# midea-ai/RDFC-GAN

Hardware: NVIDIA B200
Metric: depth maps/sec @228x304 (higher is better)
Workload: dtype bf16

## Files before the change

rdfc_gan_b200/csrc/nlspn.cu:

```cuda
#include <stdlib.h>

#include <cuda_fp16.h>

#include "common.cuh"

namespace rdfc {
namespace {

constexpr int TX = 32, TY = 8;

__device__ __forceinline__ float bilinear(const float *__restrict__ im, int H, int W, float y, float x) {
    if (!(y > -1.f && x > -1.f && y < (float)H && x < (float)W)) return 0.f;
    const float fy = floorf(y), fx = floorf(x);
    const int yl = (int)fy, xl = (int)fx;
    const float ly = y - fy, lx = x - fx, hy = 1.f - ly, hx = 1.f - lx;
    const bool y0 = yl >= 0, y1 = yl + 1 <= H - 1, x0 = xl >= 0, x1 = xl + 1 <= W - 1;
    const float *r0 = im + (long long)yl * W + xl;
    const float v1 = (y0 && x0) ? __ldg(r0) : 0.f;
    const float v2 = (y0 && x1) ? __ldg(r0 + 1) : 0.f;
    const float v3 = (y1 && x0) ? __ldg(r0 + W) : 0.f;
    const float v4 = (y1 && x1) ? __ldg(r0 + W + 1) : 0.f;
    return hy * hx * v1 + hy * lx * v2 + ly * hx * v3 + ly * lx * v4;
}

template <bool kPacked>
__global__ void __launch_bounds__(TX *TY) nlspn_affinity_kernel(const float *__restrict__ guidance,
                                                                const float *__restrict__ confidence,
                                                                const float *__restrict__ conv_w,
                                                                const float *__restrict__ conv_b,
                                                                const float *__restrict__ aff_scale, int affinity,
                                                                int conf_prop, float *__restrict__ offset,
                                                                float *__restrict__ aff, uint4 *__restrict__ packed, int H, int W) {
    __shared__ __align__(16) float s_w[72 * 24];
    __shared__ float s_b[24];
    __shared__ float s_g[8][TY + 2][TX + 2];
    const int tid = threadIdx.y * TX + threadIdx.x;
    const int b = blockIdx.z, x0 = blockIdx.x * TX, y0 = blockIdx.y * TY;
    const long long P = (long long)H * W;
    for (int e = tid; e < 24 * 72; e += TX * TY) s_w[(e % 72) * 24 + e / 72] = conv_w[e];
    if (tid < 24) s_b[tid] = conv_b[tid];
    for (int e = tid; e < 8 * (TY + 2) * (TX + 2); e += TX * TY) {
        const int c = e / ((TY + 2) * (TX + 2)), r = e % ((TY + 2) * (TX + 2));
        const int yy = y0 + r / (TX + 2) - 1, xx = x0 + r % (TX + 2) - 1;
        s_g[c][r / (TX + 2)][r % (TX + 2)] =
            (yy >= 0 && yy < H && xx >= 0 && xx < W) ? __ldg(guidance + ((long long)b * 8 + c) * P + (long long)yy * W + xx) : 0.f;
    }
    __syncthreads();
    const int x = x0 + threadIdx.x, y = y0 + threadIdx.y;
    if (x >= W || y >= H) return;

    float o[24];
#pragma unroll
    for (int c = 0; c < 24; ++c) o[c] = s_b[c];
#pragma unroll
    for (int ci = 0; ci < 8; ++ci)
#pragma unroll
        for (int t = 0; t < 9; ++t) {
            const float g = s_g[ci][threadIdx.y + t / 3][threadIdx.x + t % 3];
            const float4 *w4 = reinterpret_cast<const float4 *>(s_w + (ci * 9 + t) * 24);
#pragma unroll
            for (int c4 = 0; c4 < 6; ++c4) {
                const float4 w = w4[c4];
                o[4 * c4 + 0] = fmaf(w.x, g, o[4 * c4 + 0]);
                o[4 * c4 + 1] = fmaf(w.y, g, o[4 * c4 + 1]);
                o[4 * c4 + 2] = fmaf(w.z, g, o[4 * c4 + 2]);
                o[4 * c4 + 3] = fmaf(w.w, g, o[4 * c4 + 3]);
            }
        }

    const float scale = __ldg(aff_scale);
    float a[8];
    float abs_sum = 0.f;
    const float *conf = confidence + (long long)b * P;
#pragma unroll
    for (int j = 0; j < 8; ++j) {
        float v = o[16 + j];
        if (affinity == RDFC_AFF_TC) v = tanhf(v) / scale;
        else if (affinity == RDFC_AFF_TGASS) v = tanhf(v) / (scale + 1e-8f);
        if (conf_prop) v *= bilinear(conf, H, W, (float)y + o[2 * j], (float)x + o[2 * j + 1]);
        a[j] = v;
        abs_sum += fabsf(v);
    }
    abs_sum += 1e-4f;
    if (affinity == RDFC_AFF_ASS || affinity == RDFC_AFF_TGASS) abs_sum = abs_sum < 1.f ? 1.f : abs_sum;
    float sum = 0.f;
#pragma unroll
    for (int j = 0; j < 8; ++j) {
        if (affinity != RDFC_AFF_TC) a[j] = a[j] / abs_sum;
        sum += a[j];
    }
    const long long pix = (long long)y * W + x;
    if (kPacked) {
        const long long g = (long long)b * P + pix;
        uint4 *p = packed + (g >> 5) * 96 + (g & 31);
        auto h2 = [](float a_, float b_) { const __half2 h = __floats2half2_rn(a_, b_); return *reinterpret_cast<const uint32_t *>(&h); };
        p[0] = make_uint4(h2(o[0], o[1]), h2(o[2], o[3]), h2(o[4], o[5]), h2(o[6], o[7]));
        p[32] = make_uint4(h2(o[8], o[9]), h2(o[10], o[11]), h2(o[12], o[13]), h2(o[14], o[15]));
        p[64] = make_uint4(h2(a[0], a[1]), h2(a[2], a[3]), h2(a[4], a[5]), h2(a[6], a[7]));
        return;
    }
    float *offp = offset + (long long)b * 18 * P + pix;
    float *affp = aff + (long long)b * 9 * P + pix;
#pragma unroll
    for (int j = 0; j < 8; ++j) {
        const int k = j < 4 ? j : j + 1;
        offp[(long long)(2 * k) * P] = o[2 * j];
        offp[(long long)(2 * k + 1) * P] = o[2 * j + 1];
        affp[(long long)k * P] = a[j];
    }
    offp[8 * P] = 0.f;
    offp[9 * P] = 0.f;
    affp[4 * P] = 1.f - sum;
}

struct FuseOut { const float *d1, *c1, *c2; float *pred; };

__device__ __forceinline__ float feat_at(const float *__restrict__ im, const float *__restrict__ fix, long long i) {
    float v = __ldg(im + i);
    if (fix) {
        const float f = __ldg(fix + i);
        v = f > 0.f ? f : v;
    }
    return v;
}

__device__ __forceinline__ float bilinear_fix(const float *__restrict__ im, const float *__restrict__ fix, int H, int W, float y, float x) {
    if (!(y > -1.f && x > -1.f && y < (float)H && x < (float)W)) return 0.f;
    const float fy = floorf(y), fx = floorf(x);
    const int yl = (int)fy, xl = (int)fx;
    const float ly = y - fy, lx = x - fx, hy = 1.f - ly, hx = 1.f - lx;
    const bool y0 = yl >= 0, y1 = yl + 1 <= H - 1, x0 = xl >= 0, x1 = xl + 1 <= W - 1;
    const long long i = (long long)yl * W + xl;
    const float v1 = (y0 && x0) ? feat_at(im, fix, i) : 0.f;
    const float v2 = (y0 && x1) ? feat_at(im, fix, i + 1) : 0.f;
    const float v3 = (y1 && x0) ? feat_at(im, fix, i + W) : 0.f;
    const float v4 = (y1 && x1) ? feat_at(im, fix, i + W + 1) : 0.f;
    return hy * hx * v1 + hy * lx * v2 + ly * hx * v3 + ly * lx * v4;
}

struct BandView {
    const float *tile;
    const float *im, *fix;
    int pitch, ty0, nrows, H, W;
    float Hf, Wf;
};

template <typename FDy, typename FDx, typename FA>
__device__ __forceinline__ float gather9(const BandView &v, FDy dyf, FDx dxf, FA af, int y, int x) {
    float ymin = 1e30f, ymax = -1e30f;
#pragma unroll
    for (int k = 0; k < 9; ++k) {
        const float cy = fminf(fmaxf((float)(y - 1 + k / 3) + dyf(k), -1.f), v.Hf);
        ymin = fminf(ymin, cy);
        ymax = fmaxf(ymax, cy);
    }
    const bool esc = ((int)floorf(ymin) < v.ty0) | ((int)floorf(ymax) + 1 >= v.ty0 + v.nrows);
    float acc = 0.f;
    if (!esc) {
#pragma unroll
        for (int k = 0; k < 9; ++k) {
            const float cy = fminf(fmaxf((float)(y - 1 + k / 3) + dyf(k), -1.f), v.Hf);
            const float cx = fminf(fmaxf((float)(x - 1 + k % 3) + dxf(k), -1.f), v.Wf);
            const float fy = floorf(cy), fx = floorf(cx);
            const float ly = cy - fy, lx = cx - fx, hy = 1.f - ly, hx = 1.f - lx;
            const float *q = v.tile + (int)fmaf(fy - (float)v.ty0, (float)v.pitch, fx + 1.f);
            acc = fmaf(af(k), hy * hx * q[0] + hy * lx * q[1] + ly * hx * q[v.pitch] + ly * lx * q[v.pitch + 1], acc);
        }
    } else {
#pragma unroll
        for (int k = 0; k < 9; ++k)
            acc = fmaf(af(k), bilinear_fix(v.im, v.fix, v.H, v.W, (float)(y - 1 + k / 3) + dyf(k), (float)(x - 1 + k % 3) + dxf(k)), acc);
    }
    return acc;
}

constexpr int BAND_THREADS = 256;

__device__ __forceinline__ void stage_band(float *tile, const float *__restrict__ im, const float *__restrict__ fix, int ty0, int nrows,
                                           int pitch, int H, int W) {
    const int warp = threadIdx.x >> 5, lane = threadIdx.x & 31;
    for (int tr = warp; tr < nrows; tr += BAND_THREADS / 32) {
        const int iy = ty0 + tr;
        const bool yok = iy >= 0 && iy < H;
        const long long base = (long long)iy * W - 1;
        float *dst = tile + tr * pitch;
        for (int tc = lane; tc < pitch; tc += 32) dst[tc] = (yok && tc >= 1 && tc <= W) ? feat_at(im, fix, base + tc) : 0.f;
    }
}

template <bool kFinal>
__device__ __forceinline__ float finish(float acc, int clamp, const FuseOut &fz, long long o) {
    if (kFinal) {
        if (clamp) acc = fminf(fmaxf(acc, -1.f), 1.f);
        if (fz.pred) {
            const float a = __ldg(fz.c1 + o), b = __ldg(fz.c2 + o), m = fmaxf(a, b);
            const float e1 = expf(a - m), e2 = expf(b - m), inv = 1.f / (e1 + e2);
            fz.pred[o] = __ldg(fz.d1 + o) * (e1 * inv) + acc * (e2 * inv);
        }
    }
    return acc;
}

__device__ __forceinline__ float ld_stream(const float *p) {
    float v;
    asm volatile("ld.global.nc.L1::no_allocate.f32 %0, [%1];" : "=f"(v) : "l"(p));
    return v;
}
__device__ __forceinline__ float2 ld_stream2(const float *p) {
    float2 v;
    asm volatile("ld.global.nc.L1::no_allocate.v2.f32 {%0, %1}, [%2];" : "=f"(v.x), "=f"(v.y) : "l"(p));
    return v;
}
__device__ __forceinline__ uint4 ld_stream4(const uint4 *p) {
    uint4 v;
    asm volatile("ld.global.nc.L1::no_allocate.v4.u32 {%0, %1, %2, %3}, [%4];" : "=r"(v.x), "=r"(v.y), "=r"(v.z), "=r"(v.w) : "l"(p));
    return v;
}

template <bool kFinal, int kPix, int kMinBlocks>
__global__ void __launch_bounds__(BAND_THREADS, kMinBlocks)
nlspn_prop_band_kernel(const float *__restrict__ in, const float *__restrict__ offset, const float *__restrict__ aff,
                       const float *__restrict__ fixp, float *__restrict__ out, float *__restrict__ inter, FuseOut fz, int clamp,
                       int B, int H, int W, int rows_per_cta, int sub_rows, int halo, int pitch) {
    extern __shared__ float band_tile[];
    const long long total = (long long)B * H, P = (long long)H * W;
    long long row = (long long)blockIdx.x * rows_per_cta;
    const long long row_end = row + rows_per_cta < total ? row + rows_per_cta : total;
    const int Wp = W / kPix;
    const float Hf = (float)H, Wf = (float)W;
    asm volatile("griddepcontrol.launch_dependents;" ::: "memory");
    asm volatile("griddepcontrol.wait;" ::: "memory");
    while (row < row_end) {
        const int b = (int)(row / H), y_lo = (int)(row - (long long)b * H);
        long long nrl = row_end - row;
        if (nrl > H - y_lo) nrl = H - y_lo;
        if (nrl > sub_rows) nrl = sub_rows;
        const int nr = (int)nrl;
        const int ty0 = y_lo - halo - 1;
        const int nrows = nr + 2 * halo + 3;
        const float *im = in + (long long)b * P;
        const float *fix = fixp ? fixp + (long long)b * P : nullptr;
        __syncthreads();
        stage_band(band_tile, im, fix, ty0, nrows, pitch, H, W);
        __syncthreads();
        const BandView bv{band_tile, im, fix, pitch, ty0, nrows, H, W, Hf, Wf};
        const int nitems = nr * Wp;
        for (int idx = threadIdx.x; idx < nitems; idx += BAND_THREADS) {
            const int ry = idx / Wp, x = kPix * (idx - ry * Wp), y = y_lo + ry;
            const long long pix = (long long)y * W + x;
            const float *offp = offset + (long long)b * 18 * P + pix;
            const float *affp = aff + (long long)b * 9 * P + pix;
            const long long o = (long long)b * P + pix;
            if (kPix == 2) {
                float2 a[9], dy[9], dx[9];
#pragma unroll
                for (int k = 0; k < 9; ++k) {
                    a[k] = ld_stream2(affp + (long long)k * P);
                    if (k == 4) {
                        dy[k] = dx[k] = make_float2(0.f, 0.f);
                    } else {
                        dy[k] = ld_stream2(offp + (long long)(2 * k) * P);
                        dx[k] = ld_stream2(offp + (long long)(2 * k + 1) * P);
                    }
                }
                float acc0 = gather9(bv, [&](int k) { return dy[k].x; }, [&](int k) { return dx[k].x; }, [&](int k) { return a[k].x; }, y, x);
                float acc1 = gather9(bv, [&](int k) { return dy[k].y; }, [&](int k) { return dx[k].y; }, [&](int k) { return a[k].y; }, y, x + 1);
                acc0 = finish<kFinal>(acc0, clamp, fz, o);
                acc1 = finish<kFinal>(acc1, clamp, fz, o + 1);
                *reinterpret_cast<float2 *>(out + o) = make_float2(acc0, acc1);
                if (inter) *reinterpret_cast<float2 *>(inter + o) = make_float2(acc0, acc1);
            } else {
                float a[9], dy[9], dx[9];
#pragma unroll
                for (int k = 0; k < 9; ++k) {
                    a[k] = ld_stream(affp + (long long)k * P);
                    if (k == 4) {
                        dy[k] = dx[k] = 0.f;
                    } else {
                        dy[k] = ld_stream(offp + (long long)(2 * k) * P);
                        dx[k] = ld_stream(offp + (long long)(2 * k + 1) * P);
                    }
                }
                float acc = gather9(bv, [&](int k) { return dy[k]; }, [&](int k) { return dx[k]; }, [&](int k) { return a[k]; }, y, x);
                acc = finish<kFinal>(acc, clamp, fz, o);
                out[o] = acc;
                if (inter) inter[o] = acc;
            }
        }
        row += nr;
    }
}

__device__ __forceinline__ float2 h2f(uint32_t u) {
    const __half2 h = *reinterpret_cast<const __half2 *>(&u);
    return __half22float2(h);
}

template <bool kFinal>
__global__ void __launch_bounds__(BAND_THREADS, 4)
nlspn_prop_packed_kernel(const float *__restrict__ in, const uint4 *__restrict__ pk, const float *__restrict__ fixp,
                         float *__restrict__ out, FuseOut fz, int clamp, int B, int H, int W, int rows_per_cta, int sub_rows, int halo, int pitch) {
    extern __shared__ float band_tile[];
    const long long total = (long long)B * H, P = (long long)H * W;
    long long row = (long long)blockIdx.x * rows_per_cta;
    const long long row_end = row + rows_per_cta < total ? row + rows_per_cta : total;
    const float Hf = (float)H, Wf = (float)W;
    asm volatile("griddepcontrol.launch_dependents;" ::: "memory");
    asm volatile("griddepcontrol.wait;" ::: "memory");
    while (row < row_end) {
        const int b = (int)(row / H), y_lo = (int)(row - (long long)b * H);
        long long nrl = row_end - row;
        if (nrl > H - y_lo) nrl = H - y_lo;
        if (nrl > sub_rows) nrl = sub_rows;
        const int nr = (int)nrl;
        const int ty0 = y_lo - halo - 1;
        const int nrows = nr + 2 * halo + 3;
        const float *im = in + (long long)b * P;
        const float *fix = fixp ? fixp + (long long)b * P : nullptr;
        __syncthreads();
        stage_band(band_tile, im, fix, ty0, nrows, pitch, H, W);
        __syncthreads();
        const BandView bv{band_tile, im, fix, pitch, ty0, nrows, H, W, Hf, Wf};
        const long long g0 = (long long)b * P + (long long)y_lo * W, g1 = g0 + (long long)nr * W;
        long long g = (g0 & ~31ll) + threadIdx.x;
        uint4 n0 = make_uint4(0, 0, 0, 0), n1 = n0, n2 = n0;
        if (g < g1) { const uint4 *p = pk + (g >> 5) * 96 + (g & 31); n0 = ld_stream4(p); n1 = ld_stream4(p + 32); n2 = ld_stream4(p + 64); }
        for (; g < g1; g += BAND_THREADS) {
            const uint4 c0 = n0, c1 = n1, c2 = n2;
            if (g + BAND_THREADS < g1) {
                const uint4 *p = pk + ((g + BAND_THREADS) >> 5) * 96 + ((g + BAND_THREADS) & 31);
                n0 = ld_stream4(p); n1 = ld_stream4(p + 32); n2 = ld_stream4(p + 64);
            }
            if (g < g0) continue;
            const int pix = (int)(g - (long long)b * P), y = pix / W, x = pix - y * W;
            float dy[9], dx[9], a[9];
            {
                float2 t;
                t = h2f(c0.x); dy[0] = t.x; dx[0] = t.y;
                t = h2f(c0.y); dy[1] = t.x; dx[1] = t.y;
                t = h2f(c0.z); dy[2] = t.x; dx[2] = t.y;
                t = h2f(c0.w); dy[3] = t.x; dx[3] = t.y;
                dy[4] = dx[4] = 0.f;
                t = h2f(c1.x); dy[5] = t.x; dx[5] = t.y;
                t = h2f(c1.y); dy[6] = t.x; dx[6] = t.y;
                t = h2f(c1.z); dy[7] = t.x; dx[7] = t.y;
                t = h2f(c1.w); dy[8] = t.x; dx[8] = t.y;
                t = h2f(c2.x); a[0] = t.x; a[1] = t.y;
                t = h2f(c2.y); a[2] = t.x; a[3] = t.y;
                t = h2f(c2.z); a[5] = t.x; a[6] = t.y;
                t = h2f(c2.w); a[7] = t.x; a[8] = t.y;
                a[4] = 1.f - (((a[0] + a[1]) + (a[2] + a[3])) + ((a[5] + a[6]) + (a[7] + a[8])));
            }
            float acc = gather9(bv, [&](int k) { return dy[k]; }, [&](int k) { return dx[k]; }, [&](int k) { return a[k]; }, y, x);
            acc = finish<kFinal>(acc, clamp, fz, g);
            out[g] = acc;
        }
        row += nr;
    }
}

template <bool kFinal>
__global__ void __launch_bounds__(TX *TY) nlspn_prop_kernel(const float *__restrict__ in, const float *__restrict__ offset,
                                                            const float *__restrict__ aff, const float *__restrict__ fixp,
                                                            float *__restrict__ out, float *__restrict__ inter, FuseOut fz, int clamp,
                                                            int H, int W) {
    const int x = blockIdx.x * TX + threadIdx.x, y = blockIdx.y * TY + threadIdx.y, b = blockIdx.z;
    if (x >= W || y >= H) return;
    const long long P = (long long)H * W, pix = (long long)y * W + x;
    const float *offp = offset + (long long)b * 18 * P + pix;
    const float *affp = aff + (long long)b * 9 * P + pix;
    const float *im = in + (long long)b * P;
    const float *fix = fixp ? fixp + (long long)b * P : nullptr;
    float dy[9], dx[9], a[9];
#pragma unroll
    for (int k = 0; k < 9; ++k) {
        a[k] = ld_stream(affp + (long long)k * P);
        dy[k] = k == 4 ? 0.f : ld_stream(offp + (long long)(2 * k) * P);
        dx[k] = k == 4 ? 0.f : ld_stream(offp + (long long)(2 * k + 1) * P);
    }
    float acc = 0.f;
#pragma unroll
    for (int k = 0; k < 9; ++k)
        acc = fmaf(a[k], bilinear_fix(im, fix, H, W, (float)(y - 1 + k / 3) + dy[k], (float)(x - 1 + k % 3) + dx[k]), acc);
    acc = finish<kFinal>(acc, clamp, fz, (long long)b * P + pix);
    out[(long long)b * P + pix] = acc;
    if (inter) inter[(long long)b * P + pix] = acc;
}

__global__ void fuse_depth_kernel(const float *__restrict__ d1, const float *__restrict__ c1,
                                  const float *__restrict__ d2, const float *__restrict__ c2,
                                  float *__restrict__ d2c, float *__restrict__ pred, size_t n) {
    for (size_t i = (size_t)blockIdx.x * blockDim.x + threadIdx.x; i < n; i += (size_t)gridDim.x * blockDim.x) {
        const float v2 = fminf(fmaxf(d2[i], -1.f), 1.f);
        const float a = c1[i], b = c2[i], m = fmaxf(a, b);
        const float e1 = expf(a - m), e2 = expf(b - m), inv = 1.f / (e1 + e2);
        if (d2c) d2c[i] = v2;
        pred[i] = d1[i] * (e1 * inv) + v2 * (e2 * inv);
    }
}

static int band_pitch(int W) { return knob("RDFC_NLSPN_PITCH32", 1) != 0 ? (W + 4 + 31) / 32 * 32 : W + 4; }

struct BandGeom { int per_sm, rows_per_cta, sub_rows, nctas; size_t smem; bool ok; };
static BandGeom band_geom(int B, int H, int W, int halo, int per_sm_max) {
    BandGeom g{};
    const long long total = (long long)B * H;
    const size_t row_bytes = (size_t)band_pitch(W) * sizeof(float);
    for (int per_sm = per_sm_max; per_sm >= 1; --per_sm) {
        const size_t cap = (size_t)(220 * 1024) / per_sm - 1024;
        int fit = (int)(cap / row_bytes) - 2 * halo - 3;
        if (const long long sub = knob("RDFC_NLSPN_SUB", 0); sub > 0 && fit > sub && per_sm == per_sm_max) fit = (int)sub;
        if (fit < (per_sm > 1 && knob("RDFC_NLSPN_SUB", 0) <= 0 ? 12 : 1)) continue;
        long long ctas = (long long)sm_count() * per_sm;
        if (ctas > total) ctas = total;
        g.per_sm = per_sm;
        g.rows_per_cta = (int)((total + ctas - 1) / ctas);
        g.sub_rows = fit < g.rows_per_cta ? fit : g.rows_per_cta;
        if (g.sub_rows > H) g.sub_rows = H;
        g.nctas = (int)((total + g.rows_per_cta - 1) / g.rows_per_cta);
        g.smem = (size_t)(g.sub_rows + 2 * halo + 3) * row_bytes;
        g.ok = true;
        return g;
    }
    return g;
}

template <typename Kern, typename... Args>
static cudaError_t launch_pdl(Kern kern, int grid, int block, size_t smem, cudaStream_t st, int pdl, Args... args) {
    cudaLaunchConfig_t cfg = {};
    cfg.gridDim = dim3(grid); cfg.blockDim = dim3(block); cfg.dynamicSmemBytes = smem; cfg.stream = st;
    cudaLaunchAttribute attr[1];
    attr[0].id = cudaLaunchAttributeProgrammaticStreamSerialization;
    attr[0].val.programmaticStreamSerializationAllowed = pdl;
    cfg.attrs = attr; cfg.numAttrs = 1;
    return cudaLaunchKernelEx(&cfg, kern, args...);
}

static size_t packed_bytes(int B, int H, int W) { return (size_t)(((long long)B * H * W + 31) / 32) * 1536; }

}
}

using namespace rdfc;

static int affinity_check(const void *guidance, const void *confidence, const void *conv_w, const void *conv_b, const void *aff_scale,
                          int affinity, int conf_prop, int B, int H, int W) {
    RDFC_REQUIRE(guidance && conv_w && conv_b && aff_scale, "NULL pointer argument");
    RDFC_REQUIRE(!conf_prop || confidence, "conf_prop requires a confidence map (nlspn_model.py:150-151)");
    RDFC_REQUIRE(B > 0 && H > 0 && W > 0 && B <= 65535, "bad shape (%d,%d,%d)", B, H, W);
    RDFC_REQUIRE(affinity >= RDFC_AFF_AS && affinity <= RDFC_AFF_TGASS, "unknown affinity mode %d", affinity);
    return 0;
}

extern "C" int rdfc_nlspn_affinity_forward(const float *guidance, const float *confidence, const float *conv_w,
                                           const float *conv_b, const float *aff_scale, int affinity, int conf_prop,
                                           float *offset, float *aff, int B, int H, int W, void *stream) {
    if (int rc = affinity_check(guidance, confidence, conv_w, conv_b, aff_scale, affinity, conf_prop, B, H, W)) return rc;
    RDFC_REQUIRE(offset && aff, "NULL output pointer");
    dim3 grid(cdiv(W, TX), cdiv(H, TY), B), block(TX, TY);
    nlspn_affinity_kernel<false><<<grid, block, 0, (cudaStream_t)stream>>>(guidance, confidence, conv_w, conv_b, aff_scale,
                                                                            affinity, conf_prop, offset, aff, nullptr, H, W);
    RDFC_CHECK_LAUNCH("nlspn_affinity_kernel");
    return 0;
}

extern "C" size_t rdfc_nlspn_packed_bytes(int B, int H, int W) { return (B > 0 && H > 0 && W > 0) ? packed_bytes(B, H, W) : 0; }

extern "C" int rdfc_nlspn_affinity_forward_packed(const float *guidance, const float *confidence, const float *conv_w,
                                                  const float *conv_b, const float *aff_scale, int affinity, int conf_prop,
                                                  void *packed, int B, int H, int W, void *stream) {
    if (int rc = affinity_check(guidance, confidence, conv_w, conv_b, aff_scale, affinity, conf_prop, B, H, W)) return rc;
    RDFC_REQUIRE(packed && ((uintptr_t)packed % 16) == 0, "packed stream must be a 16-byte aligned buffer of rdfc_nlspn_packed_bytes()");
    dim3 grid(cdiv(W, TX), cdiv(H, TY), B), block(TX, TY);
    nlspn_affinity_kernel<true><<<grid, block, 0, (cudaStream_t)stream>>>(guidance, confidence, conv_w, conv_b, aff_scale,
                                                                           affinity, conf_prop, nullptr, nullptr, (uint4 *)packed, H, W);
    RDFC_CHECK_LAUNCH("nlspn_affinity_kernel");
    return 0;
}

static int propagate(const float *feat_init, const float *offset, const float *aff, const void *packed, const float *feat_fix,
                     int preserve_input, float *out, float *scratch, float *inter, int B, int H, int W, int prop_time, int clamp_out,
                     const rdfc_fuse_out *fuse, cudaStream_t st) {
    RDFC_REQUIRE(feat_init && out && scratch, "NULL pointer argument");
    RDFC_REQUIRE(!preserve_input || feat_fix, "preserve_input requires feat_fix (nlspn_model.py:157-158)");
    RDFC_REQUIRE(B > 0 && H > 0 && W > 0 && prop_time >= 0, "bad shape (%d,%d,%d) x %d", B, H, W, prop_time);
    RDFC_REQUIRE(!fuse || (fuse->d1 && fuse->c1 && fuse->c2 && fuse->pred), "fuse: NULL pointer");
    const long long P = (long long)H * W;
    const FuseOut fz = fuse ? FuseOut{fuse->d1, fuse->c1, fuse->c2, fuse->pred} : FuseOut{nullptr, nullptr, nullptr, nullptr};
    const int clamp = (clamp_out || fuse) ? 1 : 0;
    if (prop_time == 0) {
        if (fuse) {
            const int nblk = (int)min((long long)cdiv(B * P, 256), (long long)sm_count() * 8);
            fuse_depth_kernel<<<nblk, 256, 0, st>>>(fuse->d1, fuse->c1, feat_init, fuse->c2, out, fuse->pred, (size_t)(B * P));
            RDFC_CHECK_LAUNCH("fuse_depth_kernel");
        } else {
            RDFC_CUDA(cudaMemcpyAsync(out, feat_init, sizeof(float) * B * P, cudaMemcpyDeviceToDevice, st));
        }
        return 0;
    }
    const float *fix = preserve_input ? feat_fix : nullptr;
    const int halo = (int)knob("RDFC_NLSPN_HALO", 6);
    const int pdl = knob("RDFC_NLSPN_PDL", 1) != 0;
    const bool simple = knob("RDFC_NLSPN_SIMPLE", 0) != 0;
    const int pix = (!packed && W % 2 == 0 && P % 2 == 0 && ((uintptr_t)offset % 8) == 0 && ((uintptr_t)aff % 8) == 0 &&
                     ((uintptr_t)out % 8) == 0 && ((uintptr_t)scratch % 8) == 0 && (!inter || ((uintptr_t)inter % 8) == 0)) ? 2 : 1;
    const int per_sm_max = (int)knob("RDFC_NLSPN_PER_SM", packed ? 4 : (pix == 2 ? 3 : 5));
    const BandGeom g = band_geom(B, H, W, halo, per_sm_max);
    const bool band = g.ok && !simple;
    RDFC_REQUIRE(band || !packed, "packed NLSPN stream: image too wide for the band kernel (W = %d)", W);
    if (band) {
        if (packed) {
            RDFC_CUDA(cudaFuncSetAttribute(nlspn_prop_packed_kernel<false>, cudaFuncAttributeMaxDynamicSharedMemorySize, 220 * 1024));
            RDFC_CUDA(cudaFuncSetAttribute(nlspn_prop_packed_kernel<true>, cudaFuncAttributeMaxDynamicSharedMemorySize, 220 * 1024));
        } else if (pix == 2) {
            RDFC_CUDA(cudaFuncSetAttribute(nlspn_prop_band_kernel<false, 2, 3>, cudaFuncAttributeMaxDynamicSharedMemorySize, 220 * 1024));
            RDFC_CUDA(cudaFuncSetAttribute(nlspn_prop_band_kernel<true, 2, 3>, cudaFuncAttributeMaxDynamicSharedMemorySize, 220 * 1024));
        } else {
            RDFC_CUDA(cudaFuncSetAttribute(nlspn_prop_band_kernel<false, 1, 5>, cudaFuncAttributeMaxDynamicSharedMemorySize, 220 * 1024));
            RDFC_CUDA(cudaFuncSetAttribute(nlspn_prop_band_kernel<true, 1, 5>, cudaFuncAttributeMaxDynamicSharedMemorySize, 220 * 1024));
        }
    }
    float *bufs[2] = {scratch, out};
    const float *cur = feat_init;
    for (int t = 0; t < prop_time; ++t) {
        float *dst = bufs[(prop_time - 1 - t) % 2 == 0 ? 1 : 0];
        float *it = inter ? inter + (long long)t * B * P : nullptr;
        const bool last = t == prop_time - 1;
        const FuseOut none{nullptr, nullptr, nullptr, nullptr};
        if (band && packed) {
            if (last) RDFC_CUDA(launch_pdl(nlspn_prop_packed_kernel<true>, g.nctas, BAND_THREADS, g.smem, st, pdl, cur, (const uint4 *)packed, fix, dst, fz, clamp, B, H, W, g.rows_per_cta, g.sub_rows, halo, band_pitch(W)));
            else RDFC_CUDA(launch_pdl(nlspn_prop_packed_kernel<false>, g.nctas, BAND_THREADS, g.smem, st, pdl, cur, (const uint4 *)packed, fix, dst, none, 0, B, H, W, g.rows_per_cta, g.sub_rows, halo, band_pitch(W)));
            RDFC_CHECK_LAUNCH("nlspn_prop_packed_kernel");
        } else if (band) {
#define RDFC_BAND(FIN, PX, MB, FZ, CL)                                                                                            \
    RDFC_CUDA(launch_pdl(nlspn_prop_band_kernel<FIN, PX, MB>, g.nctas, BAND_THREADS, g.smem, st, pdl, cur, offset, aff, fix, dst, it, \
                         FZ, CL, B, H, W, g.rows_per_cta, g.sub_rows, halo, band_pitch(W)))
            if (pix == 2) { if (last) RDFC_BAND(true, 2, 3, fz, clamp); else RDFC_BAND(false, 2, 3, none, 0); }
            else { if (last) RDFC_BAND(true, 1, 5, fz, clamp); else RDFC_BAND(false, 1, 5, none, 0); }
#undef RDFC_BAND
            RDFC_CHECK_LAUNCH("nlspn_prop_band_kernel");
        } else {
            RDFC_REQUIRE(B <= 65535, "batch too large for the fallback kernel");
            dim3 grid(cdiv(W, TX), cdiv(H, TY), B), block(TX, TY);
            if (last) nlspn_prop_kernel<true><<<grid, block, 0, st>>>(cur, offset, aff, fix, dst, it, fz, clamp, H, W);
            else nlspn_prop_kernel<false><<<grid, block, 0, st>>>(cur, offset, aff, fix, dst, it, none, 0, H, W);
            RDFC_CHECK_LAUNCH("nlspn_prop_kernel");
        }
        cur = dst;
    }
    return 0;
}

extern "C" int rdfc_nlspn_propagate_forward(const float *feat_init, const float *offset, const float *aff,
                                            const float *feat_fix, int preserve_input, float *out, float *scratch,
                                            float *inter, int B, int H, int W, int prop_time, int clamp_out,
                                            const rdfc_fuse_out *fuse, void *stream) {
    RDFC_REQUIRE(offset && aff, "NULL pointer argument");
    return propagate(feat_init, offset, aff, nullptr, feat_fix, preserve_input, out, scratch, inter, B, H, W, prop_time, clamp_out,
                     fuse, (cudaStream_t)stream);
}

extern "C" int rdfc_nlspn_propagate_forward_packed(const float *feat_init, const void *packed, const float *feat_fix,
                                                   int preserve_input, float *out, float *scratch, int B, int H, int W,
                                                   int prop_time, int clamp_out, const rdfc_fuse_out *fuse, void *stream) {
    RDFC_REQUIRE(packed && ((uintptr_t)packed % 16) == 0, "packed stream must be 16-byte aligned");
    return propagate(feat_init, nullptr, nullptr, packed, feat_fix, preserve_input, out, scratch, nullptr, B, H, W, prop_time,
                     clamp_out, fuse, (cudaStream_t)stream);
}

__global__ void __launch_bounds__(TX *TY) nlspn_affinity_bwd_kernel(const float *__restrict__ guidance, const float *__restrict__ confidence,
                                                                    const float *__restrict__ conv_w, const float *__restrict__ conv_b,
                                                                    const float *__restrict__ aff_scale, int affinity, int conf_prop,
                                                                    const float *__restrict__ offset, const float *__restrict__ g_offset,
                                                                    const float *__restrict__ g_aff, float *__restrict__ g_conv,
                                                                    float *__restrict__ g_conf, float *__restrict__ g_scale, int H, int W) {
    __shared__ __align__(16) float s_w[72 * 8];
    __shared__ float s_b[8];
    __shared__ float s_g[8][TY + 2][TX + 2];
    __shared__ float s_red[TX * TY / 32];
    const int tid = threadIdx.y * TX + threadIdx.x;
    const int b = blockIdx.z, x0 = blockIdx.x * TX, y0 = blockIdx.y * TY;
    const long long P = (long long)H * W;
    for (int e = tid; e < 8 * 72; e += TX * TY) s_w[(e % 72) * 8 + e / 72] = conv_w[16 * 72 + e];
    if (tid < 8) s_b[tid] = conv_b[16 + tid];
    for (int e = tid; e < 8 * (TY + 2) * (TX + 2); e += TX * TY) {
        const int c = e / ((TY + 2) * (TX + 2)), r = e % ((TY + 2) * (TX + 2));
        const int yy = y0 + r / (TX + 2) - 1, xx = x0 + r % (TX + 2) - 1;
        s_g[c][r / (TX + 2)][r % (TX + 2)] =
            (yy >= 0 && yy < H && xx >= 0 && xx < W) ? __ldg(guidance + ((long long)b * 8 + c) * P + (long long)yy * W + xx) : 0.f;
    }
    __syncthreads();
    const int x = x0 + threadIdx.x, y = y0 + threadIdx.y;
    const bool live = x < W && y < H;
    float gs = 0.f;
    if (live) {
        float r[8];
#pragma unroll
        for (int j = 0; j < 8; ++j) r[j] = s_b[j];
#pragma unroll
        for (int ci = 0; ci < 8; ++ci)
#pragma unroll
            for (int t = 0; t < 9; ++t) {
                const float g = s_g[ci][threadIdx.y + t / 3][threadIdx.x + t % 3];
                const float4 *w4 = reinterpret_cast<const float4 *>(s_w + (ci * 9 + t) * 8);
                const float4 w0 = w4[0], w1 = w4[1];
                r[0] = fmaf(w0.x, g, r[0]); r[1] = fmaf(w0.y, g, r[1]); r[2] = fmaf(w0.z, g, r[2]); r[3] = fmaf(w0.w, g, r[3]);
                r[4] = fmaf(w1.x, g, r[4]); r[5] = fmaf(w1.y, g, r[5]); r[6] = fmaf(w1.z, g, r[6]); r[7] = fmaf(w1.w, g, r[7]);
            }
        const long long pix = (long long)y * W + x;
        const float *offp = offset + (long long)b * 18 * P + pix;
        const float *gop = g_offset + (long long)b * 18 * P + pix;
        const float *gap = g_aff + (long long)b * 9 * P + pix;
        float *gc = g_conv + (long long)b * 24 * P + pix;
        const float scale = __ldg(aff_scale);
        const float den = affinity == RDFC_AFF_TGASS ? scale + 1e-8f : scale;
        const float *conf = conf_prop ? confidence + (long long)b * P : nullptr;
        float t[8], v[8], c[8], u[8], dy[8], dx[8];
        float abs_sum = 0.f;
#pragma unroll
        for (int j = 0; j < 8; ++j) {
            const int k = j < 4 ? j : j + 1;
            dy[j] = __ldg(offp + (long long)(2 * k) * P);
            dx[j] = __ldg(offp + (long long)(2 * k + 1) * P);
            t[j] = (affinity == RDFC_AFF_TC || affinity == RDFC_AFF_TGASS) ? tanhf(r[j]) : r[j];
            v[j] = (affinity == RDFC_AFF_TC || affinity == RDFC_AFF_TGASS) ? t[j] / den : r[j];
            c[j] = conf_prop ? bilinear(conf, H, W, (float)y + dy[j], (float)x + dx[j]) : 1.f;
            u[j] = v[j] * c[j];
            abs_sum += fabsf(u[j]);
        }
        abs_sum += 1e-4f;
        bool clamped = false;
        if ((affinity == RDFC_AFF_ASS || affinity == RDFC_AFF_TGASS) && abs_sum < 1.f) { abs_sum = 1.f; clamped = true; }
        const float g_ref = __ldg(gap + 4 * P);
        float ga[8], dot = 0.f;
#pragma unroll
        for (int j = 0; j < 8; ++j) {
            const int k = j < 4 ? j : j + 1;
            ga[j] = __ldg(gap + (long long)k * P) - g_ref;
            dot += ga[j] * u[j];
        }
#pragma unroll
        for (int j = 0; j < 8; ++j) {
            float gu = ga[j];
            if (affinity != RDFC_AFF_TC) {
                const float sgn = u[j] > 0.f ? 1.f : (u[j] < 0.f ? -1.f : 0.f);
                gu = ga[j] / abs_sum - (clamped ? 0.f : dot / (abs_sum * abs_sum) * sgn);
            }
            const float gv = gu * c[j];
            if (conf_prop) {
                const float gcj = gu * v[j], sy = (float)y + dy[j], sx = (float)x + dx[j];
                if (gcj != 0.f && sy > -1.f && sx > -1.f && sy < (float)H && sx < (float)W) {
                    const float fy = floorf(sy), fx = floorf(sx);
                    const int yl = (int)fy, xl = (int)fx;
                    const float ly = sy - fy, lx = sx - fx;
                    float *gim = g_conf + (long long)b * P;
#pragma unroll
                    for (int aa = 0; aa < 2; ++aa)
#pragma unroll
                        for (int cc = 0; cc < 2; ++cc) {
                            const int yy = yl + aa, xx = xl + cc;
                            if (yy >= 0 && yy <= H - 1 && xx >= 0 && xx <= W - 1)
                                atomicAdd(gim + (long long)yy * W + xx, (aa ? ly : 1.f - ly) * (cc ? lx : 1.f - lx) * gcj);
                        }
                }
            }
            float gr = gv;
            if (affinity == RDFC_AFF_TC || affinity == RDFC_AFF_TGASS) {
                gr = gv * (1.f - t[j] * t[j]) / den;
                gs -= gv * t[j] / (den * den);
            }
            gc[(long long)(16 + j) * P] = gr;
            const int k = j < 4 ? j : j + 1;
            gc[(long long)(2 * j) * P] = __ldg(gop + (long long)(2 * k) * P);
            gc[(long long)(2 * j + 1) * P] = __ldg(gop + (long long)(2 * k + 1) * P);
        }
    }
    if (g_scale) {
        for (int o = 16; o > 0; o >>= 1) gs += __shfl_down_sync(0xffffffffu, gs, o);
        if ((tid & 31) == 0) s_red[tid >> 5] = gs;
        __syncthreads();
        if (tid == 0) {
            float tot = 0.f;
            for (int w = 0; w < TX * TY / 32; ++w) tot += s_red[w];
            if (tot != 0.f) atomicAdd(g_scale, tot);
        }
    }
}

struct BwdPos { int yl, xl; float ly, lx; bool valid; };
__device__ __forceinline__ BwdPos bwd_pos(float y, float x, int H, int W) {
    BwdPos q;
    q.valid = y > -1.f && x > -1.f && y < (float)H && x < (float)W;
    const float yf = floorf(y), xf = floorf(x);
    q.yl = (int)yf; q.xl = (int)xf; q.ly = y - yf; q.lx = x - xf;
    return q;
}

__global__ void __launch_bounds__(256) nlspn_bwd_scatter_kernel(float *__restrict__ g, const float *__restrict__ ginter,
                                                                const float *__restrict__ fix, const float *__restrict__ offset,
                                                                const float *__restrict__ aff, float *__restrict__ gprev,
                                                                int finalize, int H, int W) {
    const long long P = (long long)H * W;
    const int b = blockIdx.y;
    const long long pix = (long long)blockIdx.x * 256 + threadIdx.x;
    if (pix >= P) return;
    const long long o = (long long)b * P + pix;
    float gv = g[o];
    if (finalize) {
        if (fix && __ldg(fix + o) > 0.f) gv = 0.f;
        if (ginter) gv += __ldg(ginter + o);
        g[o] = gv;
    }
    if (gv == 0.f) return;
    const int y = (int)(pix / W), x = (int)(pix - (long long)y * W);
    const float *offp = offset + (long long)b * 18 * P + pix;
    const float *affp = aff + (long long)b * 9 * P + pix;
    float *gim = gprev + (long long)b * P;
#pragma unroll
    for (int k = 0; k < 9; ++k) {
        const float sy = (float)(y - 1 + k / 3) + __ldg(offp + (long long)(2 * k) * P);
        const float sx = (float)(x - 1 + k % 3) + __ldg(offp + (long long)(2 * k + 1) * P);
        const BwdPos q = bwd_pos(sy, sx, H, W);
        if (!q.valid) continue;
        const float top = gv * __ldg(affp + (long long)k * P);
#pragma unroll
        for (int a = 0; a < 2; ++a)
#pragma unroll
            for (int c = 0; c < 2; ++c) {
                const int yy = q.yl + a, xx = q.xl + c;
                if (yy >= 0 && yy <= H - 1 && xx >= 0 && xx <= W - 1)
                    atomicAdd(gim + (long long)yy * W + xx, (a ? q.ly : 1.f - q.ly) * (c ? q.lx : 1.f - q.lx) * top);
            }
    }
}

template <bool kPreserve>
__global__ void __launch_bounds__(256) nlspn_bwd_coord_kernel(const float *__restrict__ feat_init, const float *__restrict__ inter,
                                                              const float *__restrict__ fix, const float *__restrict__ G,
                                                              const float *__restrict__ offset, const float *__restrict__ aff,
                                                              float *__restrict__ goff, float *__restrict__ gaff,
                                                              int B, int H, int W, int T) {
    const long long P = (long long)H * W, BP = (long long)B * P;
    const int b = blockIdx.y;
    const long long pix = (long long)blockIdx.x * 256 + threadIdx.x;
    if (pix >= P) return;
    const long long o = (long long)b * P + pix;
    const int y = (int)(pix / W), x = (int)(pix - (long long)y * W);
    const float *offp = offset + (long long)b * 18 * P + pix;
    const float *affp = aff + (long long)b * 9 * P + pix;
    const float *fx = kPreserve ? fix + (long long)b * P : nullptr;
#pragma unroll 1
    for (int k = 0; k < 9; ++k) {
        const float sy = (float)(y - 1 + k / 3) + __ldg(offp + (long long)(2 * k) * P);
        const float sx = (float)(x - 1 + k % 3) + __ldg(offp + (long long)(2 * k + 1) * P);
        const float m = __ldg(affp + (long long)k * P);
        float a_m = 0.f, a_y = 0.f, a_x = 0.f;
        if (!(sy <= -1.f || sy >= (float)H || sx <= -1.f || sx >= (float)W)) {
            const BwdPos q = bwd_pos(sy, sx, H, W);
            const int yh = q.yl + 1, xh = q.xl + 1;
            const bool ok1 = q.yl >= 0 && q.xl >= 0, ok2 = q.yl >= 0 && xh <= W - 1, ok3 = yh <= H - 1 && q.xl >= 0,
                       ok4 = yh <= H - 1 && xh <= W - 1;
            const long long i1 = (long long)q.yl * W + q.xl, i2 = i1 + 1, i3 = i1 + W, i4 = i3 + 1;
            const float hy = 1.f - q.ly, hx = 1.f - q.lx;
            for (int t = 1; t <= T; ++t) {
                const float gv = __ldg(G + (long long)t * BP + o);
                if (gv == 0.f) continue;
                const float *im = (t == 1 ? feat_init : inter + (long long)(t - 2) * BP) + (long long)b * P;
                float v1 = ok1 ? __ldg(im + i1) : 0.f, v2 = ok2 ? __ldg(im + i2) : 0.f, v3 = ok3 ? __ldg(im + i3) : 0.f,
                      v4 = ok4 ? __ldg(im + i4) : 0.f;
                if (kPreserve) {
                    const float f1 = ok1 ? __ldg(fx + i1) : 0.f, f2 = ok2 ? __ldg(fx + i2) : 0.f, f3 = ok3 ? __ldg(fx + i3) : 0.f,
                                f4 = ok4 ? __ldg(fx + i4) : 0.f;
                    v1 = f1 > 0.f ? f1 : v1; v2 = f2 > 0.f ? f2 : v2; v3 = f3 > 0.f ? f3 : v3; v4 = f4 > 0.f ? f4 : v4;
                }
                const float val = hy * hx * v1 + hy * q.lx * v2 + q.ly * hx * v3 + q.ly * q.lx * v4;
                a_m += gv * val;
// ... 82 lines not shown
```

Before: 2957.

## Use packed FP32x2 math in NLSPN affinity conv and deformable gather paths

The affinity kernel now computes two pixels per thread with paired FFMA2 instructions, and it prefetches weights and guidance into registers before writing them to shared memory. The propagation gather adds a fast path for when all vertical offsets fall within the halo, which skips the band-escape min/max check. That path samples two taps at once using packed float2 add/multiply and a magic-number floor. Band staging is batched so several loads are in flight per lane. These changes cut instruction count and load latency, in exchange for more register pressure and integer-bit tricks in floor/address computation that could be fragile at edge values.

```diff
diff --git a/rdfc_gan_b200/csrc/nlspn.cu b/rdfc_gan_b200/csrc/nlspn.cu
--- a/rdfc_gan_b200/csrc/nlspn.cu
+++ b/rdfc_gan_b200/csrc/nlspn.cu
@@ -23,6 +23,60 @@
     return hy * hx * v1 + hy * lx * v2 + ly * hx * v3 + ly * lx * v4;
 }
 
+constexpr int AX = 2 * TX;
+
+template <bool kPacked>
+__device__ __forceinline__ void affinity_epilogue(const float2 (&o2)[12], const float *__restrict__ conf, float scale, int affinity,
+                                                  int conf_prop, float *__restrict__ offset, float *__restrict__ aff,
+                                                  uint4 *__restrict__ packed, int b, int H, int W, int y, int x, bool store) {
+    const long long P = (long long)H * W;
+    float o[24];
+#pragma unroll
+    for (int c = 0; c < 12; ++c) { o[2 * c] = o2[c].x; o[2 * c + 1] = o2[c].y; }
+    float a[8];
+    float abs_sum = 0.f;
+#pragma unroll
+    for (int j = 0; j < 8; ++j) {
+        float v = o[16 + j];
+        if (affinity == RDFC_AFF_TC) v = tanhf(v) / scale;
+        else if (affinity == RDFC_AFF_TGASS) v = tanhf(v) / (scale + 1e-8f);
+        if (conf_prop) v *= bilinear(conf, H, W, (float)y + o[2 * j], (float)x + o[2 * j + 1]);
+        a[j] = v;
+        abs_sum += fabsf(v);
+    }
+    abs_sum += 1e-4f;
+    if (affinity == RDFC_AFF_ASS || affinity == RDFC_AFF_TGASS) abs_sum = abs_sum < 1.f ? 1.f : abs_sum;
+    float sum = 0.f;
+#pragma unroll
+    for (int j = 0; j < 8; ++j) {
+        if (affinity != RDFC_AFF_TC) a[j] = a[j] / abs_sum;
+        sum += a[j];
+    }
+    if (!store) return;
+    const long long pix = (long long)y * W + x;
+    if (kPacked) {
+        const long long g = (long long)b * P + pix;
+        uint4 *p = packed + (g >> 5) * 96 + (g & 31);
+        auto h2 = [](float a_, float b_) { const __half2 h = __floats2half2_rn(a_, b_); return *reinterpret_cast<const uint32_t *>(&h); };
+        p[0] = make_uint4(h2(o[0], o[1]), h2(o[2], o[3]), h2(o[4], o[5]), h2(o[6], o[7]));
+        p[32] = make_uint4(h2(o[8], o[9]), h2(o[10], o[11]), h2(o[12], o[13]), h2(o[14], o[15]));
+        p[64] = make_uint4(h2(a[0], a[1]), h2(a[2], a[3]), h2(a[4], a[5]), h2(a[6], a[7]));
+        return;
+    }
+    float *offp = offset + (long long)b * 18 * P + pix;
+    float *affp = aff + (long long)b * 9 * P + pix;
+#pragma unroll
+    for (int j = 0; j < 8; ++j) {
+        const int k = j < 4 ? j : j + 1;
+        offp[(long long)(2 * k) * P] = o[2 * j];
+        offp[(long long)(2 * k + 1) * P] = o[2 * j + 1];
+        affp[(long long)k * P] = a[j];
+    }
+    offp[8 * P] = 0.f;
+    offp[9 * P] = 0.f;
+    affp[4 * P] = 1.f - sum;
+}
+
 template <bool kPacked>
 __global__ void __launch_bounds__(TX *TY) nlspn_affinity_kernel(const float *__restrict__ guidance,
                                                                 const float *__restrict__ confidence,
@@ -33,84 +87,65 @@
                                                                 float *__restrict__ aff, uint4 *__restrict__ packed, int H, int W) {
     __shared__ __align__(16) float s_w[72 * 24];
     __shared__ float s_b[24];
-    __shared__ float s_g[8][TY + 2][TX + 2];
+    __shared__ __align__(8) float s_g[8][TY + 2][AX + 2];
     const int tid = threadIdx.y * TX + threadIdx.x;
-    const int b = blockIdx.z, x0 = blockIdx.x * TX, y0 = blockIdx.y * TY;
+    const int b = blockIdx.z, x0 = blockIdx.x * AX, y0 = blockIdx.y * TY;
     const long long P = (long long)H * W;
-    for (int e = tid; e < 24 * 72; e += TX * TY) s_w[(e % 72) * 24 + e / 72] = conv_w[e];
+    constexpr int NW = 24 * 72, NG = 8 * (TY + 2) * (AX + 2), NT = TX * TY;
+    float wv[(NW + NT - 1) / NT], gv[(NG + NT - 1) / NT];
+#pragma unroll
+    for (int i = 0; i < (NW + NT - 1) / NT; ++i) wv[i] = tid + i * NT < NW ? __ldg(conv_w + tid + i * NT) : 0.f;
+#pragma unroll
+    for (int i = 0; i < (NG + NT - 1) / NT; ++i) {
+        const int e = tid + i * NT, c = e / ((TY + 2) * (AX + 2)), r = e % ((TY + 2) * (AX + 2));
+        const int yy = y0 + r / (AX + 2) - 1, xx = x0 + r % (AX + 2) - 1;
+        gv[i] = (e < NG && yy >= 0 && yy < H && xx >= 0 && xx < W) ? __ldg(guidance + ((long long)b * 8 + c) * P + (long long)yy * W + xx) : 0.f;
+    }
     if (tid < 24) s_b[tid] = conv_b[tid];
-    for (int e = tid; e < 8 * (TY + 2) * (TX + 2); e += TX * TY) {
-        const int c = e / ((TY + 2) * (TX + 2)), r = e % ((TY + 2) * (TX + 2));
-        const int yy = y0 + r / (TX + 2) - 1, xx = x0 + r % (TX + 2) - 1;
-        s_g[c][r / (TX + 2)][r % (TX + 2)] =
-            (yy >= 0 && yy < H && xx >= 0 && xx < W) ? __ldg(guidance + ((long long)b * 8 + c) * P + (long long)yy * W + xx) : 0.f;
+#pragma unroll
+    for (int i = 0; i < (NW + NT - 1) / NT; ++i) {
+        const int e = tid + i * NT;
+        if (e < NW) s_w[(e % 72) * 24 + e / 72] = wv[i];
+    }
+#pragma unroll
+    for (int i = 0; i < (NG + NT - 1) / NT; ++i) {
+        const int e = tid + i * NT;
+        if (e < NG) (&s_g[0][0][0])[e] = gv[i];
     }
     __syncthreads();
-    const int x = x0 + threadIdx.x, y = y0 + threadIdx.y;
+    const int x = x0 + 2 * threadIdx.x, y = y0 + threadIdx.y;
     if (x >= W || y >= H) return;
 
-    float o[24];
-#pragma unroll
-    for (int c = 0; c < 24; ++c) o[c] = s_b[c];
+    float2 o0[12], o1[12];
+#pragma unroll
+    for (int c = 0; c < 12; ++c) o0[c] = o1[c] = make_float2(s_b[2 * c], s_b[2 * c + 1]);
 #pragma unroll
     for (int ci = 0; ci < 8; ++ci)
 #pragma unroll
-        for (int t = 0; t < 9; ++t) {
-            const float g = s_g[ci][threadIdx.y + t / 3][threadIdx.x + t % 3];
-            const float4 *w4 = reinterpret_cast<const float4 *>(s_w + (ci * 9 + t) * 24);
-#pragma unroll
-            for (int c4 = 0; c4 < 6; ++c4) {
-                const float4 w = w4[c4];
-                o[4 * c4 + 0] = fmaf(w.x, g, o[4 * c4 + 0]);
-                o[4 * c4 + 1] = fmaf(w.y, g, o[4 * c4 + 1]);
-                o[4 * c4 + 2] = fmaf(w.z, g, o[4 * c4 + 2]);
-                o[4 * c4 + 3] = fmaf(w.w, g, o[4 * c4 + 3]);
+        for (int ky = 0; ky < 3; ++ky) {
+            const float2 *row = reinterpret_cast<const float2 *>(&s_g[ci][threadIdx.y + ky][2 * threadIdx.x]);
+            const float2 ga = row[0], gb = row[1];
+            const float g[4] = {ga.x, ga.y, gb.x, gb.y};
+#pragma unroll
+            for (int kx = 0; kx < 3; ++kx) {
+                const float4 *w4 = reinterpret_cast<const float4 *>(s_w + (ci * 9 + ky * 3 + kx) * 24);
+                const float2 g0 = make_float2(g[kx], g[kx]), g1 = make_float2(g[kx + 1], g[kx + 1]);
+#pragma unroll
+                for (int c4 = 0; c4 < 6; ++c4) {
+                    const float4 w = w4[c4];
+                    const float2 wl = make_float2(w.x, w.y), wh = make_float2(w.z, w.w);
+                    o0[2 * c4] = __ffma2_rn(wl, g0, o0[2 * c4]);
+                    o0[2 * c4 + 1] = __ffma2_rn(wh, g0, o0[2 * c4 + 1]);
+                    o1[2 * c4] = __ffma2_rn(wl, g1, o1[2 * c4]);
+                    o1[2 * c4 + 1] = __ffma2_rn(wh, g1, o1[2 * c4 + 1]);
+                }
             }
         }
 
     const float scale = __ldg(aff_scale);
-    float a[8];
-    float abs_sum = 0.f;
     const float *conf = confidence + (long long)b * P;
-#pragma unroll
-    for (int j = 0; j < 8; ++j) {
-        float v = o[16 + j];
-        if (affinity == RDFC_AFF_TC) v = tanhf(v) / scale;
-        else if (affinity == RDFC_AFF_TGASS) v = tanhf(v) / (scale + 1e-8f);
-        if (conf_prop) v *= bilinear(conf, H, W, (float)y + o[2 * j], (float)x + o[2 * j + 1]);
-        a[j] = v;
-        abs_sum += fabsf(v);
-    }
-    abs_sum += 1e-4f;
-    if (affinity == RDFC_AFF_ASS || affinity == RDFC_AFF_TGASS) abs_sum = abs_sum < 1.f ? 1.f : abs_sum;
-    float sum = 0.f;
-#pragma unroll
-    for (int j = 0; j < 8; ++j) {
-        if (affinity != RDFC_AFF_TC) a[j] = a[j] / abs_sum;
-        sum += a[j];
-    }
-    const long long pix = (long long)y * W + x;
-    if (kPacked) {
-        const long long g = (long long)b * P + pix;
-        uint4 *p = packed + (g >> 5) * 96 + (g & 31);
-        auto h2 = [](float a_, float b_) { const __half2 h = __floats2half2_rn(a_, b_); return *reinterpret_cast<const uint32_t *>(&h); };
-        p[0] = make_uint4(h2(o[0], o[1]), h2(o[2], o[3]), h2(o[4], o[5]), h2(o[6], o[7]));
-        p[32] = make_uint4(h2(o[8], o[9]), h2(o[10], o[11]), h2(o[12], o[13]), h2(o[14], o[15]));
-        p[64] = make_uint4(h2(a[0], a[1]), h2(a[2], a[3]), h2(a[4], a[5]), h2(a[6], a[7]));
-        return;
-    }
-    float *offp = offset + (long long)b * 18 * P + pix;
-    float *affp = aff + (long long)b * 9 * P + pix;
-#pragma unroll
-    for (int j = 0; j < 8; ++j) {
-        const int k = j < 4 ? j : j + 1;
-        offp[(long long)(2 * k) * P] = o[2 * j];
-        offp[(long long)(2 * k + 1) * P] = o[2 * j + 1];
-        affp[(long long)k * P] = a[j];
-    }
-    offp[8 * P] = 0.f;
-    offp[9 * P] = 0.f;
-    affp[4 * P] = 1.f - sum;
+    affinity_epilogue<kPacked>(o0, conf, scale, affinity, conf_prop, offset, aff, packed, b, H, W, y, x, true);
+    affinity_epilogue<kPacked>(o1, conf, scale, affinity, conf_prop, offset, aff, packed, b, H, W, y, x + 1, x + 1 < W);
 }
 
 struct FuseOut { const float *d1, *c1, *c2; float *pred; };
@@ -142,29 +177,61 @@
     const float *tile;
     const float *im, *fix;
     int pitch, ty0, nrows, H, W;
-    float Hf, Wf;
+    float Hf, Wf, halo;
 };
+
+constexpr float kFloorMagic = 0x1.8p23f;
+constexpr int kFloorMagicBits = 0x4B400000;
+
+__device__ __forceinline__ float2 neg2(float2 v) { return make_float2(-v.x, -v.y); }
+
+__device__ __forceinline__ float2 sample2(const BandView &v, float2 cy, float2 cx) {
+    const float2 magic = make_float2(kFloorMagic, kFloorMagic), one = make_float2(1.f, 1.f);
+    const float2 my = __fadd2_rd(cy, magic), mx = __fadd2_rd(cx, magic);
+    const float2 ly = __fadd2_rn(cy, neg2(__fadd2_rn(my, neg2(magic)))), lx = __fadd2_rn(cx, neg2(__fadd2_rn(mx, neg2(magic))));
+    const float2 hy = __fadd2_rn(one, neg2(ly)), hx = __fadd2_rn(one, neg2(lx));
+    const unsigned base = 1u - (unsigned)v.ty0 * v.pitch - (unsigned)kFloorMagicBits * (v.pitch + 1);
+    const float *q0 = v.tile + (int)(base + __float_as_uint(my.x) * v.pitch + __float_as_uint(mx.x));
+    const float *q1 = v.tile + (int)(base + __float_as_uint(my.y) * v.pitch + __float_as_uint(mx.y));
+    float2 s = __fmul2_rn(make_float2(q0[0], q1[0]), __fmul2_rn(hy, hx));
+    s = __ffma2_rn(make_float2(q0[1], q1[1]), __fmul2_rn(hy, lx), s);
+    s = __ffma2_rn(make_float2(q0[v.pitch], q1[v.pitch]), __fmul2_rn(ly, hx), s);
+    return __ffma2_rn(make_float2(q0[v.pitch + 1], q1[v.pitch + 1]), __fmul2_rn(ly, lx), s);
+}
 
 template <typename FDy, typename FDx, typename FA>
 __device__ __forceinline__ float gather9(const BandView &v, FDy dyf, FDx dxf, FA af, int y, int x) {
-    float ymin = 1e30f, ymax = -1e30f;
-#pragma unroll
-    for (int k = 0; k < 9; ++k) {
-        const float cy = fminf(fmaxf((float)(y - 1 + k / 3) + dyf(k), -1.f), v.Hf);
-        ymin = fminf(ymin, cy);
-        ymax = fmaxf(ymax, cy);
-    }
-    const bool esc = ((int)floorf(ymin) < v.ty0) | ((int)floorf(ymax) + 1 >= v.ty0 + v.nrows);
+    bool near = true;
+#pragma unroll
+    for (int k = 0; k < 9; ++k)
+        if (k != 4) near &= fabsf(dyf(k)) <= v.halo;
+    bool esc = false;
+    if (!near) {
+        float ymin = 1e30f, ymax = -1e30f;
+#pragma unroll
+        for (int k = 0; k < 9; ++k) {
+            const float cy = fminf(fmaxf((float)(y - 1 + k / 3) + dyf(k), -1.f), v.Hf);
+            ymin = fminf(ymin, cy);
+            ymax = fmaxf(ymax, cy);
+        }
+        esc = ((int)floorf(ymin) < v.ty0) | ((int)floorf(ymax) + 1 >= v.ty0 + v.nrows);
+    }
     float acc = 0.f;
     if (!esc) {
-#pragma unroll
-        for (int k = 0; k < 9; ++k) {
-            const float cy = fminf(fmaxf((float)(y - 1 + k / 3) + dyf(k), -1.f), v.Hf);
-            const float cx = fminf(fmaxf((float)(x - 1 + k % 3) + dxf(k), -1.f), v.Wf);
-            const float fy = floorf(cy), fx = floorf(cx);
-            const float ly = cy - fy, lx = cx - fx, hy = 1.f - ly, hx = 1.f - lx;
-            const float *q = v.tile + (int)fmaf(fy - (float)v.ty0, (float)v.pitch, fx + 1.f);
-            acc = fmaf(af(k), hy * hx * q[0] + hy * lx * q[1] + ly * hx * q[v.pitch] + ly * lx * q[v.pitch + 1], acc);
+        const float yf = (float)y, xf = (float)x;
+#pragma unroll
+        for (int p = 0; p < 4; ++p) {
+            const int k0 = p < 2 ? 2 * p : 2 * p + 1, k1 = k0 + 1;
+            float2 cy = __fadd2_rn(make_float2(yf + (float)(k0 / 3 - 1), yf + (float)(k1 / 3 - 1)), make_float2(dyf(k0), dyf(k1)));
+            float2 cx = __fadd2_rn(make_float2(xf + (float)(k0 % 3 - 1), xf + (float)(k1 % 3 - 1)), make_float2(dxf(k0), dxf(k1)));
+            cy = make_float2(fminf(fmaxf(cy.x, -1.f), v.Hf), fminf(fmaxf(cy.y, -1.f), v.Hf));
+            cx = make_float2(fminf(fmaxf(cx.x, -1.f), v.Wf), fminf(fmaxf(cx.y, -1.f), v.Wf));
+            const float2 s = sample2(v, cy, cx);
+            if (p == 2) {
+                acc = fmaf(af(4), v.tile[(y - v.ty0) * v.pitch + x + 1], acc);
+            }
+            acc = fmaf(af(k0), s.x, acc);
+            acc = fmaf(af(k1), s.y, acc);
         }
     } else {
 #pragma unroll
@@ -174,7 +241,36 @@
     return acc;
 }
 
+__device__ __forceinline__ float2 gather9x2(const BandView &v, const float2 *dy, const float2 *dx, const float2 *a, int y, int x) {
+    bool near = true;
+#pragma unroll
+    for (int k = 0; k < 9; ++k)
+        if (k != 4) near &= (fabsf(dy[k].x) <= v.halo) & (fabsf(dy[k].y) <= v.halo);
+    if (!near)
+        return make_float2(gather9(v, [&](int k) { return dy[k].x; }, [&](int k) { return dx[k].x; }, [&](int k) { return a[k].x; }, y, x),
+                           gather9(v, [&](int k) { return dy[k].y; }, [&](int k) { return dx[k].y; }, [&](int k) { return a[k].y; }, y, x + 1));
+    const float yf = (float)y, xf = (float)x;
+    float2 acc = make_float2(0.f, 0.f);
+#pragma unroll
+    for (int k = 0; k < 9; ++k) {
+        float2 s;
+        if (k == 4) {
+            const float *q = v.tile + (y - v.ty0) * v.pitch + x + 1;
+            s = make_float2(q[0], q[1]);
+        } else {
+            const float by = yf + (float)(k / 3 - 1), bx = xf + (float)(k % 3 - 1);
+            float2 cy = __fadd2_rn(make_float2(by, by), dy[k]), cx = __fadd2_rn(make_float2(bx, bx + 1.f), dx[k]);
+            cy = make_float2(fminf(fmaxf(cy.x, -1.f), v.Hf), fminf(fmaxf(cy.y, -1.f), v.Hf));
+            cx = make_float2(fminf(fmaxf(cx.x, -1.f), v.Wf), fminf(fmaxf(cx.y, -1.f), v.Wf));
+            s = sample2(v, cy, cx);
+        }
+        acc = __ffma2_rn(a[k], s, acc);
+    }
+    return acc;
+}
+
 constexpr int BAND_THREADS = 256;
+constexpr int kStageBatch = 8;
 
 __device__ __forceinline__ void stage_band(float *tile, const float *__restrict__ im, const float *__restrict__ fix, int ty0, int nrows,
                                            int pitch, int H, int W) {
@@ -184,7 +280,17 @@
         const bool yok = iy >= 0 && iy < H;
         const long long base = (long long)iy * W - 1;
         float *dst = tile + tr * pitch;
-        for (int tc = lane; tc < pitch; tc += 32) dst[tc] = (yok && tc >= 1 && tc <= W) ? feat_at(im, fix, base + tc) : 0.f;
+        for (int tc0 = lane; tc0 < pitch; tc0 += 32 * kStageBatch) {
+            float v[kStageBatch];
+#pragma unroll
+            for (int u = 0; u < kStageBatch; ++u) {
+                const int tc = tc0 + 32 * u;
+                v[u] = (yok && tc >= 1 && tc <= W) ? feat_at(im, fix, base + tc) : 0.f;
+            }
+#pragma unroll
+            for (int u = 0; u < kStageBatch; ++u)
+                if (tc0 + 32 * u < pitch) dst[tc0 + 32 * u] = v[u];
+        }
     }
 }
 
@@ -243,7 +349,7 @@
         __syncthreads();
         stage_band(band_tile, im, fix, ty0, nrows, pitch, H, W);
         __syncthreads();
-        const BandView bv{band_tile, im, fix, pitch, ty0, nrows, H, W, Hf, Wf};
+        const BandView bv{band_tile, im, fix, pitch, ty0, nrows, H, W, Hf, Wf, (float)halo};
         const int nitems = nr * Wp;
         for (int idx = threadIdx.x; idx < nitems; idx += BAND_THREADS) {
             const int ry = idx / Wp, x = kPix * (idx - ry * Wp), y = y_lo + ry;
@@ -263,10 +369,9 @@
                         dx[k] = ld_stream2(offp + (long long)(2 * k + 1) * P);
                     }
                 }
-                float acc0 = gather9(bv, [&](int k) { return dy[k].x; }, [&](int k) { return dx[k].x; }, [&](int k) { return a[k].x; }, y, x);
-                float acc1 = gather9(bv, [&](int k) { return dy[k].y; }, [&](int k) { return dx[k].y; }, [&](int k) { return a[k].y; }, y, x + 1);
-                acc0 = finish<kFinal>(acc0, clamp, fz, o);
-                acc1 = finish<kFinal>(acc1, clamp, fz, o + 1);
+                const float2 acc = gather9x2(bv, dy, dx, a, y, x);
+                const float acc0 = finish<kFinal>(acc.x, clamp, fz, o);
+                const float acc1 = finish<kFinal>(acc.y, clamp, fz, o + 1);
                 *reinterpret_cast<float2 *>(out + o) = make_float2(acc0, acc1);
                 if (inter) *reinterpret_cast<float2 *>(inter + o) = make_float2(acc0, acc1);
             } else {
@@ -320,7 +425,7 @@
         __syncthreads();
         stage_band(band_tile, im, fix, ty0, nrows, pitch, H, W);
         __syncthreads();
-        const BandView bv{band_tile, im, fix, pitch, ty0, nrows, H, W, Hf, Wf};
+        const BandView bv{band_tile, im, fix, pitch, ty0, nrows, H, W, Hf, Wf, (float)halo};
         const long long g0 = (long long)b * P + (long long)y_lo * W, g1 = g0 + (long long)nr * W;
         long long g = (g0 & ~31ll) + threadIdx.x;
         uint4 n0 = make_uint4(0, 0, 0, 0), n1 = n0, n2 = n0;
@@ -457,7 +562,7 @@
                                            float *offset, float *aff, int B, int H, int W, void *stream) {
     if (int rc = affinity_check(guidance, confidence, conv_w, conv_b, aff_scale, affinity, conf_prop, B, H, W)) return rc;
     RDFC_REQUIRE(offset && aff, "NULL output pointer");
-    dim3 grid(cdiv(W, TX), cdiv(H, TY), B), block(TX, TY);
+    dim3 grid(cdiv(W, AX), cdiv(H, TY), B), block(TX, TY);
     nlspn_affinity_kernel<false><<<grid, block, 0, (cudaStream_t)stream>>>(guidance, confidence, conv_w, conv_b, aff_scale,
                                                                             affinity, conf_prop, offset, aff, nullptr, H, W);
     RDFC_CHECK_LAUNCH("nlspn_affinity_kernel");
@@ -471,7 +576,7 @@
                                                   void *packed, int B, int H, int W, void *stream) {
     if (int rc = affinity_check(guidance, confidence, conv_w, conv_b, aff_scale, affinity, conf_prop, B, H, W)) return rc;
     RDFC_REQUIRE(packed && ((uintptr_t)packed % 16) == 0, "packed stream must be a 16-byte aligned buffer of rdfc_nlspn_packed_bytes()");
-    dim3 grid(cdiv(W, TX), cdiv(H, TY), B), block(TX, TY);
+    dim3 grid(cdiv(W, AX), cdiv(H, TY), B), block(TX, TY);
     nlspn_affinity_kernel<true><<<grid, block, 0, (cudaStream_t)stream>>>(guidance, confidence, conv_w, conv_b, aff_scale,
                                                                            affinity, conf_prop, nullptr, nullptr, (uint4 *)packed, H, W);
     RDFC_CHECK_LAUNCH("nlspn_affinity_kernel");
```

Result: no change. 2982 (median of 6 runs) (+0.9%).
